# miniufo/xinvert

Measured on AMD Instinct MI355X. Metric: SOR grid-points*iters/sec (fp64) at 3600x1800, masked points counted, higher is better.
Workload: dtype f64

## Files before the change

### xinvert_amd/csrc/xinv_launch.h

```cpp
#pragma once

static inline unsigned cdiv(int64_t a, int64_t b) { return (unsigned)((a + b - 1) / b); }

#if XINV_TEST_HOOKS
static thread_local int *t_hook_record = nullptr;
#endif

struct Plan {
    int path, base, seam, ncol;
    int K, RY, nsg, nrb;
    int nkc, KC;
    bool K2;
    int nsg2, nrb2, nkc2, KC2;
    int joff2;
    int cus;
    int64_t srowf2;
    bool bih_zbe;
    int bih_vm;
    bool aligned;
    unsigned umask;
    unsigned um;
    bool even_split;
    bool nine;
    bool skip;
// ... 355 lines not shown
                if (per) {
                    if (pl.umask) hipLaunchKernelGGL((k_bih_rowclass<true, true>), gb, bb, 0, st, a);
                    else          hipLaunchKernelGGL((k_bih_rowclass<false, true>), gb, bb, 0, st, a);
                } else {
                    if (pl.umask) hipLaunchKernelGGL((k_bih_rowclass<true, false>), gb, bb, 0, st, a);
                    else          hipLaunchKernelGGL((k_bih_rowclass<false, false>), gb, bb, 0, st, a);
                }
            }
            hipLaunchKernelGGL(k_rows_copy_back, dim3(256, (unsigned)nm, 1), dim3(256), 0, st,
                               (const double *)ws->S2, p.sS, p.S, p.sS, p.yc, p.xc,
                               (const XinvCtl *)ws->ctl, m0, 0);
        } else
        for (int cc = 0; cc < pl.ncol; cc++) {
            a.colour = cc;
            if (pl.umask) hipLaunchKernelGGL(k_colour_bih2d<true>, g, b, 0, st, a);
            else          hipLaunchKernelGGL(k_colour_bih2d<false>, g, b, 0, st, a);
        }
    } else if (is3d(p.kind)) {
        ColourArgs3D a;
        memset(&a, 0, sizeof a);
        a.S = p.S; a.sS = p.sS;
        for (int q = 0; q < p.ncoef; q++) { a.c[q] = p.c[q]; a.sc[q] = p.sc[q]; }
        a.zc = p.zc; a.yc = p.yc; a.xc = p.xc;
        a.per = per; a.seam = pl.seam; a.force = 0; a.sc_ = p.sc_; a.ctl = ws->ctl;
        a.nbatch = p.nbatch; a.member0 = m0;
        dim3 b(64, 4, 1);
        dim3 g(cdiv(cdiv(p.xc, 2) + 1, 64), cdiv(p.yc - 2, 4), (unsigned)(nm * (p.zc - 2)));
        for (int pos = 0; pos < pl.ncol; pos++) {
            a.colour = seam_sequence(pos, 2, pl.seam);
            if (p.kind == KIND_GEN3D) hipLaunchKernelGGL(k_colour_gen3d, g, b, 0, st, a);
            else                      hipLaunchKernelGGL(k_colour_std3d, g, b, 0, st, a);
        }
    } else {
        ColourArgs2D a;
        memset(&a, 0, sizeof a);
        a.S = p.S; a.sS = p.sS;
        for (int q = 0; q < p.ncoef; q++) { a.c[q] = p.c[q]; a.sc[q] = p.sc[q]; }
        a.yc = p.yc; a.xc = p.xc;
        a.per = per; a.base = pl.base; a.seam = pl.seam; a.force = 0;
        a.sc_ = p.sc_; a.ctl = ws->ctl; a.member0 = m0;
        dim3 b(64, 4, 1);
        dim3 g(cdiv(cdiv(p.xc, 2) + 1, 64), cdiv(p.yc - 2, 4), (unsigned)nm);
        const bool nine = (pl.base == 4);
        for (int pos = 0; pos < pl.ncol; pos++) {
            a.colour = seam_sequence(pos, pl.base, pl.seam);
            if (p.kind == KIND_STD2D) {
                if (nine) hipLaunchKernelGGL(k_colour_std2d<true>, g, b, 0, st, a);
                else      hipLaunchKernelGGL(k_colour_std2d<false>, g, b, 0, st, a);
            } else if (p.kind == KIND_STD2DT) {
                if (nine) hipLaunchKernelGGL(k_colour_std2dt<true>, g, b, 0, st, a);
                else      hipLaunchKernelGGL(k_colour_std2dt<false>, g, b, 0, st, a);
            } else {
                if (nine) hipLaunchKernelGGL(k_colour_gen2d<true>, g, b, 0, st, a);
                else      hipLaunchKernelGGL(k_colour_gen2d<false>, g, b, 0, st, a);
            }
        }
    }
    NormArgs n;
    n.S = p.S; n.sS = p.sS; n.n = p.zc * p.yc * p.xc; n.undef = p.sc_.undef;
    n.psum = (double *)ws->partials;
    n.pcnt = (long long *)((char *)ws->partials + p.nbatch * XINV_NORM_BLOCKS * sizeof(double));
    n.ctl = ws->ctl; n.stop = p.stop; n.force = 0; n.member0 = m0;
    int nblk = (int)std::min<int64_t>(XINV_NORM_BLOCKS, std::max<int64_t>(1, n.n / 2048));
    hipLaunchKernelGGL(k_norm_partial, dim3(nblk, (unsigned)nm, 1), dim3(256, 1, 1), 0, st, n);
    hipLaunchKernelGGL(k_norm_final, dim3((unsigned)nm, 1, 1), dim3(64, 1, 1), 0, st, n, nblk);
    HIPCHK(hipGetLastError());
    return XINV_OK;
}

static int launch_colour_sweep(const Problem &p, const Plan &pl, Workspace *ws, hipStream_t st)
{
    int64_t chunk = XINV_MEMBER_CHUNK;
    if (is3d(p.kind)) chunk = std::max<int64_t>(1, 65535 / std::max<int64_t>(1, p.zc - 2));
    return for_member_chunks(0, p.nbatch, [&](int64_t m0, int64_t nm) { return launch_colour_chunk(p, pl, ws, st, m0, nm); }, chunk);
}

static int pipe_occ_cap()
{
    return std::max(1, XINV_ENV_INT("XINV_PIPE_OCC", 5));
}

static double tile_cost(int64_t wgs, int64_t rows, int K, int occ, double lone, bool pipe)
{
    return xinv_tile_cost(wgs, rows, K, occ, pipe ? pipe_occ_cap() : 3, lone, pipe ? XINV_PIPE_LAG : 0);
}

static int64_t choose_row_blocks(int64_t yc, int64_t nstrip, int64_t nbatch, int K, int occ, double lone, bool pipe)
{
    return xinv_choose_row_blocks(yc, nstrip, nbatch, K, occ, pipe ? pipe_occ_cap() : 3, lone, pipe ? XINV_PIPE_LAG : 0);
}

static int plan_occ(const Problem &p, const Plan &pl, hipStream_t st, int K, bool *have = nullptr)
{
    const bool ext = (p.BCy == XINV_BC_EXTEND);
    int occ, missing;
    if (p.kind == KIND_BIH2D) {
        FusedBihArgs dummy; memset(&dummy, 0, sizeof dummy);
        occ = 1;
        missing = xinv_launch_fusedbih(false, pl.bih_zbe, pl.bih_vm, dim3(1), st, dummy, &occ);
    } else {
        FusedArgs dummy; memset(&dummy, 0, sizeof dummy);
        occ = pl.nine ? 1 : 2;
        if (pl.nine) missing = xinv_launch_fused9(p.kind == KIND_GEN2D, K, pl.aligned, ext, dim3(1), st, dummy, &occ, pl.seam != 0);
        else if (pl.pipe) missing = xinv_launch_pipe2d(p.kind == KIND_GEN2D, pl.um, pl.npair, pl.pipe_fr, pl.aligned, ext, dim3(1), st, dummy, &occ, 0, pl.seam != 0, pl.fma);
        else missing = fused_dispatch(p.kind, pl.aligned, ext, pl.um | (pl.alias_ac ? 2u : 0u), K, dim3(1), dim3(256), st, dummy, &occ, pl.seam != 0, pl.fma, pl.pq);
    }
    if (have) *have = !missing;
    return occ;
}

static void split_rows_evenly(const Problem &p, Plan &pl, int64_t nrb)
{
    pl.nrb = (int)nrb;
    pl.even_split = true;
    pl.RY = (int)cdiv(p.yc, pl.nrb);
}
static bool rows_per_tile_given(const Problem &p, const xinv_options &opt, Plan &pl)
{
    pl.even_split = false;
    if (opt.rows_per_tile > 0) {
        pl.RY = (opt.rows_per_tile + 1) & ~1;
        pl.nrb = (int)cdiv(p.yc, pl.RY);
    } else if (opt.rows_per_tile < 0)
        split_rows_evenly(p, pl, std::max<int64_t>(1, std::min<int64_t>(-opt.rows_per_tile, p.yc / 2)));
    return opt.rows_per_tile != 0;
}

static int issue_strip_active(const Problem &p, Workspace *ws, hipStream_t st, int UW, int fi)
{
    const int64_t yc = p.yc, nb = p.nbatch;
    const int nstrip = (int)cdiv(p.xc, UW);
    const int64_t cells = yc * nstrip;
    int rc = ensure_dev(&ws->d_act, &ws->d_act_cap, (size_t)(nb * cells));
    if (rc) return rc;
    if ((rc = ensure_pinned(&ws->h_act, &ws->h_act_cap, (size_t)(nb * cells), hipHostMallocDefault))) return rc;
    StripActArgs sa;
    sa.f = p.c[fi]; sa.sf = p.sc[fi]; sa.yc = yc; sa.xc = p.xc; sa.nstrip = nstrip; sa.UW = UW;
    sa.undef = p.sc_.undef; sa.act = ws->d_act;
    hipLaunchKernelGGL(k_strip_active, dim3(cdiv(cells, 4), (unsigned)nb, 1), dim3(256), 0, st, sa);
    HIPCHK(hipMemcpyAsync(ws->h_act, ws->d_act, (size_t)(nb * cells), hipMemcpyDeviceToHost, st));
    ws->act_ready = true; ws->act_uw = UW; ws->act_f = p.c[fi]; ws->act_synced = false;
    return XINV_OK;
}

static int plan_tile_skip(const Problem &p, Plan &pl, Workspace *ws, hipStream_t st,
                          const xinv_options &opt, int fixedRB = 0, int UW_ = 0)
{
    pl.skip = false; pl.ntl = pl.nskip = 0; pl.skip_pct = 0; pl.skip_ppm = 0;
    const bool forced = (opt.flags & XINV_FLAG_FORCE_TILE_SKIP) != 0;
    const int tpw = pl.pipe ? 1 : 4;
    const int K = pl.K, UW = UW_ ? UW_ : strip_uw(pl, K, pl.pipe);
    const int nstrip = (int)cdiv(p.xc, UW);
    const int64_t wscale = 4 / tpw;
    if (!forced && ((int64_t)nstrip * pl.nrb * p.nbatch * wscale < 1024 || (int64_t)nstrip * pl.nrb * wscale < 64 ||
                    p.nbatch > 64))
        return XINV_OK;
    const int64_t yc = p.yc, nb = p.nbatch;
    const int64_t cells = yc * nstrip;
    if (nb * nstrip * (yc + 1) > (int64_t)50000000) return XINV_OK;
    const StreamMap &sm = stream_map(p.kind);
    const int fi = (p.kind == KIND_BIH2D) ? 9 : sm.c[sm.forcing];

    int rc = XINV_OK;
    if (!(ws->act_ready && ws->act_uw == UW && ws->act_f == p.c[fi])) {
        rc = issue_strip_active(p, ws, st, UW, fi);
        if (rc) return rc;
        HIPCHK(hipStreamSynchronize(st));
    } else if (!ws->act_synced)
        HIPCHK(hipStreamSynchronize(st));
    ws->act_ready = false;

    std::vector<int> &pre = ws->h_pre;
    pre.resize((size_t)(nb * nstrip * (yc + 1)));
    int64_t nact = 0;
    for (int64_t m = 0; m < nb; m++) {
        int *q = &pre[(size_t)(m * (yc + 1) * nstrip)];
        for (int s = 0; s < nstrip; s++) q[s] = 0;
        const unsigned char *ha = ws->h_act + m * yc * nstrip;
        for (int64_t r = 0; r < yc; r++, q += nstrip, ha += nstrip)
            for (int s = 0; s < nstrip; s++) q[nstrip + s] = q[s] + ha[s];
        for (int s = 0; s < nstrip; s++) nact += q[s];
    }
    if (!forced && (double)nact > 0.92 * (double)(nb * cells)) return XINV_OK;
    auto rows_active = [&](int64_t m, int strip, int64_t y0, int64_t y1) {
        const int *q = &pre[(size_t)(m * (yc + 1) * nstrip)];
        return q[y1 * nstrip + strip] - q[y0 * nstrip + strip] > 0;
    };

    const bool ext = (p.BCy == XINV_BC_EXTEND);
    auto ntile_ids = [&](int nrb) { return nstrip * nrb; };
    auto id_rb = [&](int, int id) { return id / nstrip; };
    auto tile_active = [&](int64_t m, int nrb, int id) {
        const int rb = id_rb(nrb, id);
        const TileRows t = xinv_tile_rows(id, nstrip, nrb, yc, fixedRB);
        if (t.y0 >= t.y1) return false;
        if (ext && (rb == 0 || rb >= nrb - (fixedRB ? 2 : 1))) return true;
        return rows_active(m, t.strip, t.y0, t.y1);
    };
    auto active_wgs = [&](int nrb, int64_t *maxact) {
        int64_t wgs = 0, mx = 0;
        for (int64_t m = 0; m < nb; m++) {
            int64_t c = 0;
            const int *q = &pre[(size_t)(m * (yc + 1) * nstrip)];
            for (int rb = 0; rb < nrb; rb++) {
                const TileRows t = xinv_tile_rows(rb * nstrip, nstrip, nrb, yc, fixedRB);
                if (t.y0 >= t.y1) continue;
                if (ext && (rb == 0 || rb >= nrb - (fixedRB ? 2 : 1))) { c += nstrip; continue; }
                const int *q0 = q + t.y0 * nstrip, *q1 = q + t.y1 * nstrip;
                for (int st_ = 0; st_ < nstrip; st_++) c += (q1[st_] - q0[st_]) > 0;
            }
            wgs += cdiv(c, tpw); mx = std::max(mx, c);
        }
        if (maxact) *maxact = mx;
        return wgs;
    };
    const int occ = fixedRB ? 2 : plan_occ(p, pl, st, K);
    const bool pp = pl.pipe;
    const double cost0 = tile_cost((int64_t)cdiv((int64_t)nstrip * pl.nrb, tpw) * nb, cdiv(yc, pl.nrb), K, occ, pl.lone, pp);
    int best = pl.nrb; double best_cost = 1e300;
    int lo = pl.nrb, hi = pl.nrb;
    if (!forced && opt.rows_per_tile == 0 && !fixedRB) {
        const int64_t w0 = active_wgs(pl.nrb, nullptr);
        const double share = std::max(0.05, (double)w0 / (double)((int64_t)cdiv((int64_t)nstrip * pl.nrb, tpw) * nb));
        const double centre = (double)pl.nrb / share;
        const int64_t cap_rows = std::max<int64_t>(pl.nrb, yc / 4);
        lo = (int)std::min<int64_t>(cap_rows, std::max<int64_t>(pl.nrb, (int64_t)(centre * 0.85)));
        hi = (int)std::min<int64_t>(cap_rows, std::max<int64_t>(lo, (int64_t)(centre * 1.10) + 1));
    }
    best_cost = tile_cost(active_wgs(pl.nrb, nullptr), cdiv(yc, pl.nrb), K, occ, pl.lone, pp);
    for (int nrb = lo; nrb <= hi; nrb++) {
        const double c = tile_cost(active_wgs(nrb, nullptr), cdiv(yc, nrb), K, occ, pl.lone, pp);
        if (c < best_cost) { best_cost = c; best = nrb; }
    }
    if (!forced && best_cost > 0.95 * cost0) return XINV_OK;

    int64_t maxact = 0;
    active_wgs(best, &maxact);
    const int64_t ntiles = (int64_t)ntile_ids(best);
    const int ntl = (int)(tpw * std::max<int64_t>(1, cdiv(maxact, tpw)));
    int64_t maxskip = 0, nskipped = 0;
    std::vector<std::vector<int>> act((size_t)nb), skp((size_t)nb);
    for (int64_t m = 0; m < nb; m++) {
        for (int id = 0; id < (int)ntiles; id++) {
            const TileRows t = xinv_tile_rows(id, nstrip, best, yc, fixedRB);
            if (t.y0 >= t.y1) continue;
            (tile_active(m, best, id) ? act[(size_t)m] : skp[(size_t)m]).push_back(id);
        }
        maxskip = std::max<int64_t>(maxskip, (int64_t)skp[(size_t)m].size());
        nskipped += (int64_t)skp[(size_t)m].size();
    }
    if (nskipped == 0) return XINV_OK;
    const int nskip = (int)maxskip;
    const size_t nints = (size_t)nb * ((size_t)ntl + nskip);
    rc = ensure_dev(&ws->d_list, &ws->d_list_cap, nints * sizeof(int));
    if (rc) return rc;
    if ((rc = ensure_pinned(&ws->h_list, &ws->h_list_cap, nints * sizeof(int), hipHostMallocDefault))) return rc;
    int *hl = ws->h_list, *hs = ws->h_list + (size_t)nb * ntl;
    for (int64_t m = 0; m < nb; m++) {
        std::vector<int> &am = act[(size_t)m];
        if (pl.seam && !fixedRB) {
            auto heavy = [&](int id) { const int s_ = id % nstrip; return s_ == 0 || s_ == nstrip - 1; };
            const int nh = (int)(std::stable_partition(am.begin(), am.end(), heavy) - am.begin());
            const int nwg = ntl / tpw, q = nwg >> 3, rem = nwg & 7;
            for (int L = 0; L < nwg; L++) {
                const int xcd = L & 7, T = xcd * q + std::min(xcd, rem) + (L >> 3);
                const int sq = xinv_heavy_first(L, nwg, nh / tpw);
                for (int w = 0; w < tpw; w++)
                    hl[m * ntl + T * tpw + w] = sq * tpw + w < (int)am.size() ? am[(size_t)(sq * tpw + w)] : -1;
            }
        } else
        for (int t = 0; t < ntl; t++) hl[m * ntl + t] = t < (int)am.size() ? am[(size_t)t] : -1;
        for (int t = 0; t < nskip; t++) hs[m * nskip + t] = t < (int)skp[(size_t)m].size() ? skp[(size_t)m][t] : -1;
    }
    HIPCHK(hipMemcpyAsync(ws->d_list, ws->h_list, nints * sizeof(int), hipMemcpyHostToDevice, st));
    rc = ensure_dev(&ws->d_tsum, &ws->d_tsum_cap, tsum_layout(nullptr, nb, nskip).bytes);
    if (rc) return rc;
    const TsumPtrs ts = tsum_layout(ws->d_tsum, nb, nskip);
    HIPCHK(hipMemsetAsync(ts.ticket, 0, (size_t)nb * sizeof(unsigned), st));
    SkipNormArgs na;
    na.S = p.S; na.sS = p.sS; na.yc = yc; na.xc = p.xc; na.nstrip = nstrip; na.nrb = best; na.UW = UW; na.RB = fixedRB;
    na.undef = p.sc_.undef; na.skip_list = ws->d_list + (size_t)nb * ntl; na.nskip_max = nskip;
    na.tsum = ts.tsum; na.tcnt = ts.tcnt; na.xsum = ts.xsum; na.xcnt = ts.xcnt; na.ticket = ts.ticket;
    pl.skipna = na;

    pl.skip = true; pl.ntl = ntl; pl.nskip = nskip;
    pl.skip_pct = (int)((100 * nskipped) / (ntiles * nb));
    pl.skip_ppm = (int)((1000000 * nskipped) / (ntiles * nb));
    if (!fixedRB) {
        split_rows_evenly(p, pl, best);
        pl.nsg = (int)cdiv((int64_t)cdiv(p.xc, 128 - (pl.nine ? 8 : 4) * XINV_KMAX - (pl.seam ? 4 : 0)) * pl.nrb, pl.pipe ? 4 : tpw) + 1;
        if (pl.pipe) pl.nsg = std::max(pl.nsg, (int)cdiv(p.xc, UW) * pl.nrb + 1);
    }
    return XINV_OK;
}

static int detect_xuniform(Workspace *ws, hipStream_t st, const double *const *arr,
                           const int64_t *stride, int nstream, int64_t nbatch, int64_t rows,
                           int64_t xc, unsigned *mask)
{
    XUniArgs xa;
    memset(&xa, 0, sizeof xa);
    xa.nstream = nstream;
    for (int q = 0; q < nstream; q++) { xa.c[q] = arr[q]; xa.stride[q] = stride[q]; }
    xa.nbatch = nbatch; xa.yc = rows; xa.xc = xc;
    if (!ws->dflags16) {
        HIPCHK(hipMalloc((void **)&ws->dflags16, 16 * sizeof(int)));
        HIPCHK(hipHostMalloc((void **)&ws->hflags16, 16 * sizeof(int), hipHostMallocDefault));
    }
    xa.flag = ws->dflags16;
    HIPCHK(hipMemsetAsync(ws->dflags16, 0, 16 * sizeof(int), st));
    hipLaunchKernelGGL(k_xuniform, dim3(512, (unsigned)nstream, 1), dim3(256), 0, st, xa);
    HIPCHK(hipMemcpyAsync(ws->hflags16, ws->dflags16, 16 * sizeof(int), hipMemcpyDeviceToHost, st));
    HIPCHK(hipStreamSynchronize(st));
    ws->act_synced = true;
// ... 27 lines not shown
```

### xinvert_amd/csrc/xinv_pipe2d.h

```cpp
#pragma once
#include "xinv_fused.h"

#define XINV_PIPE_P 4
#ifndef XINV_PIPE_B
#define XINV_PIPE_B 2
#endif
#define XINV_PIPE_LAG (XINV_PIPE_B + 5)
#define XINV_PIPE_NS 4
#define XINV_PIPE_UW(np) (128 * (np) - 4 * XINV_PIPE_P)
#ifndef XINV_PIPE_PF0
#define XINV_PIPE_PF0 4
#endif
#ifndef XINV_PIPE_PF
#define XINV_PIPE_PF 4
#endif

template <class M, unsigned UM> struct PipeRec {
    static constexpr int NCO = M::NC - 1;
    static constexpr int NUNI = __builtin_popcount(UM & ((1u << NCO) - 1u));
    static constexpr bool HOIST = M::template hoist<UM>();
    static constexpr int NW = NUNI + (HOIST ? 2 : 0);
    static constexpr int RW = NW == 0 ? 0 : (NW <= 4 ? 4 : 8);
};

// ... 74 lines not shown
        a.q[m * a.n + t] = q;
    }
    if (__any(zero) && (threadIdx.x & 63) == 0) atomicOr(a.flag, 1);
    if (__any(differ) && (threadIdx.x & 63) == 0) atomicOr(a.flag, 2);
}
#endif

__device__ __forceinline__ void xinv_pipe_barrier()
{
    asm volatile("s_waitcnt lgkmcnt(0)\n\ts_barrier" ::: "memory");
}

typedef const double __attribute__((address_space(4))) *xinv_cdouble_ptr;
typedef const char __attribute__((address_space(1))) *xinv_gcptr;
typedef char __attribute__((address_space(1))) *xinv_gptr;
typedef double xinv_v2d __attribute__((ext_vector_type(2)));
typedef const xinv_v2d __attribute__((address_space(1))) *xinv_gcd2ptr;
typedef const double __attribute__((address_space(1))) *xinv_gcdptr;
typedef xinv_v2d __attribute__((address_space(1))) *xinv_gd2ptr;
typedef double __attribute__((address_space(1))) *xinv_gdptr;

__device__ __forceinline__ void pipe_extend_fix(double2 &edge, const double2 &inner, double inner_w,
                                                const LaneCols &lc, bool tall, double u)
{
    if (lc.cls_x == 1) { if (inner.x != u) edge.x = inner.x; }
    else if (lc.cls_x == 2) { if (inner.y != u) edge.x = inner.y; }
    else if (lc.cls_x == 3) {
        if (tall && inner.x != u) edge.x = inner.x;
        if (inner_w != u) edge.x = inner_w;
    }
    if (lc.cls_y == 1) { if (inner.y != u) edge.y = inner.y; }
    else if (lc.cls_y == 3) {
        if (tall && inner.y != u) edge.y = inner.y;
        if (inner.x != u) edge.y = inner.x;
    }
}

template <class M, unsigned UM, bool FR, int NP, bool AL, bool EXT, int PW, int PF, bool SEAM = false>
__device__ __forceinline__ void xinv_pipe_wave(const FusedArgs &a, int64_t m, int yu0, int yu1,
                                               const LaneCols (&lc)[NP], const int64_t (&st0)[NP], int lane,
                                               double2 (*ring)[XINV_PIPE_NS][NP * (FR ? 2 : 1)][XINV_WAVE], int gtot,
                                               double &acc, int &cnt,
                                               unsigned long long seam_lanes = 0ull)
{
    constexpr int P = XINV_PIPE_P, H = 2 * P, D = 4, LAG = XINV_PIPE_LAG, B = XINV_PIPE_B;
    constexpr int R = PF + D;
    constexpr int PFR = M::PIPE_PFR;
    using REC = PipeRec<M, UM>;
    constexpr int NC = M::NC, FQ = M::NC - 1, RW = REC::RW;
    constexpr bool HOIST = REC::HOIST;
    constexpr int RS = FR ? 2 : 1;
    static_assert(R % D == 0 && R % B == 0 && R % XINV_PIPE_NS == 0,
                  "the unroll period must keep row parity, ring slots and barriers compile-time");
    const int ycr = (int)a.yc;
    const unsigned rowbytes = (unsigned)a.xc * 8u;
    const double u = a.sc_.undef;
    const int slice_bytes = (int)(rowbytes * (unsigned)ycr);
    const __amdgpu_buffer_rsrc_t rsS = __builtin_amdgcn_make_buffer_rsrc((void *)(a.src + m * a.sS), 0, slice_bytes, 0x00020000);
    const __amdgpu_buffer_rsrc_t rsD = __builtin_amdgcn_make_buffer_rsrc((void *)(a.dst + m * a.sS), 0, slice_bytes, 0x00020000);
    __amdgpu_buffer_rsrc_t rsC[NC];
#pragma unroll
    for (int q = 0; q < NC; q++)
        rsC[q] = __builtin_amdgcn_make_buffer_rsrc((void *)(a.c[q] + m * a.sc[q]), 0, slice_bytes, 0x00020000);
    const xinv_cdouble_ptr rowf = (xinv_cdouble_ptr)(uintptr_t)(reinterpret_cast<const double *>(a.rowf) + m * a.yc * RW);
    unsigned lo0[NP], lo1[NP], so0[NP], so1[NP];
#pragma unroll
    for (int q = 0; q < NP; q++) {
        lo0[q] = (unsigned)lc[q].l0 * 8u; lo1[q] = (unsigned)lc[q].l1 * 8u;
        so0[q] = lc[q].use_x ? (unsigned)st0[q] * 8u : 0xffffffffu;
        so1[q] = lc[q].use_y ? (unsigned)(st0[q] + 1) * 8u : 0xffffffffu;
    }

    unsigned long long okx64[NP], oky64[NP];
    double nsx[NP], nsy[NP];
    int nnx[NP], nny[NP];
#pragma unroll
    for (int q = 0; q < NP; q++) {
        okx64[q] = __builtin_amdgcn_ballot_w64(lc[q].ok_x) & ~seam_lanes; oky64[q] = __builtin_amdgcn_ballot_w64(lc[q].ok_y);
        nsx[q] = nsy[q] = 0.0; nnx[q] = nny[q] = 0;
    }
    static_assert(!SEAM || (NP == 1 && !AL && PipeRec<M, UM>::HOIST),
                  "seam variants: one column pair per lane, per-row records, updates under EXEC masks");

    const int in_lo = yu0 - H + 2 * PW;
    const int in_hi = yu1 - 1 + H - 2 * PW;

    double2 sw[NP][R];
    CoefWin<NC, R> cw[NP];
    double rokw[R];
#pragma unroll
    for (int t = 0; t < R; t++) {
        rokw[t] = 0.0;
#pragma unroll
        for (int q = 0; q < NP; q++) {
            sw[q][t] = make_double2(0.0, 0.0);
            cw[q].rq[t] = 0.0; cw[q].mx[t] = 0u; cw[q].my[t] = 0u;
#pragma unroll
            for (int c = 0; c < NC; c++) { cw[q].v[c][t] = make_double2(0.0, 0.0); cw[q].s[c][t] = 0.0; }
        }
    }

    const int maxo = (int)(rowbytes * (unsigned)(ycr - 1));
    int nxo = (yu0 - H + 2 * PW) * (int)rowbytes;
    int nxr = (yu0 - H + 2 * PW) * (RW * 8);
    auto ldrow = [&](__amdgpu_buffer_rsrc_t rs, int soff, auto qtag) {
        constexpr int q = decltype(qtag)::value;
        double2 v;
        if (AL) {
            const auto t = __builtin_amdgcn_raw_buffer_load_b128(rs, (int)lo0[q], soff, 0);
            v.x = __hiloint2double((int)t[1], (int)t[0]); v.y = __hiloint2double((int)t[3], (int)t[2]);
        } else {
            const auto t0 = __builtin_amdgcn_raw_buffer_load_b64(rs, (int)lo0[q], soff, 0);
            const auto t1 = __builtin_amdgcn_raw_buffer_load_b64(rs, (int)lo1[q], soff, 0);
            v.x = __hiloint2double((int)t0[1], (int)t0[0]); v.y = __hiloint2double((int)t1[1], (int)t1[0]);
        }
        return v;
    };
    auto request = [&](int, auto stag) {
        constexpr int slot = decltype(stag)::value;
        const int soff = min(max(nxo, 0), maxo);
        nxo += (int)rowbytes;
        asm("" : "+s"(nxo));
        xinv_unroll_steps([&](auto qtag) {
            constexpr int q = decltype(qtag)::value;
            if (PW == 0) sw[q][slot] = ldrow(rsS, soff, qtag);
            xinv_unroll_steps([&](auto ctag) {
                constexpr int c = decltype(ctag)::value;
                if (!((UM >> c) & 1u) && !(FR && c == FQ && PW > 0)) cw[q].v[c][slot] = ldrow(rsC[c], soff, qtag);
            }, std::make_integer_sequence<int, NC>{});
        }, std::make_integer_sequence<int, NP>{});
    };
    auto request_rf = [&](int, auto stag) {
        constexpr int slot = decltype(stag)::value;
        if constexpr (RW > 0) {
            const unsigned roff = (unsigned)min(max(nxr, 0), (ycr - 1) * (RW * 8));
            nxr += RW * 8;
            const xinv_cdouble_ptr pr = (xinv_cdouble_ptr)((const char __attribute__((address_space(4))) *)rowf + roff);
            double rec[RW];
#pragma unroll
            for (int k = 0; k < RW; k++) rec[k] = pr[k];
#pragma unroll
            for (int q = 0; q < NP; q++) {
                int k = 0;
#pragma unroll
                for (int c = 0; c < NC - 1; c++)
                    if ((UM >> c) & 1u) cw[q].s[c][slot] = rec[k++];
                if (HOIST) { cw[q].rq[slot] = rec[k]; rokw[slot] = rec[k + 1]; }
            }
        }
    };
    xinv_unroll_steps([&](auto ttag) { request(in_lo + decltype(ttag)::value, ttag); asm volatile("" ::: "memory"); },
                      std::make_integer_sequence<int, PF>{});
    xinv_unroll_steps([&](auto ttag) { request_rf(in_lo + decltype(ttag)::value, ttag); },
                      std::make_integer_sequence<int, PFR>{});

    auto half_pass = [&](auto xtag, auto jtag, auto ptag, auto mtag, auto fixt) {
        constexpr int X = decltype(xtag)::value, sj = decltype(jtag)::value, sjp = decltype(ptag)::value,
                      sjm = decltype(mtag)::value;
        constexpr bool FIX = decltype(fixt)::value;
        static_assert(!FIX || (X == 0 && NP == 1), "column xc-1 sits in an .x slot");
        const double edge = (X == 0) ? xinv_lane_up(sw[NP - 1][sj].y) : xinv_lane_down(sw[0][sj].x);
        double nv[NP];
#pragma unroll
        for (int q = 0; q < NP; q++) {
            double w, e;
            if (X == 0) { w = (q == 0) ? edge : sw[q > 0 ? q - 1 : 0][sj].y; e = sw[q][sj].y; }
            else        { w = sw[q][sj].x; e = (q == NP - 1) ? edge : sw[q < NP - 1 ? q + 1 : q][sj].x; }
            if constexpr (FIX) e = xinv_lane_down(sw[q][sj].x);
            const double t = M::template inc<X, UM, R, false>(cw[q], sj, sjp, comp<X>(sw[q][sj]), comp<X>(sw[q][sjp]),
                                              comp<X>(sw[q][sjm]), w, e, a.sc_);
            if constexpr (HOIST) {
                const unsigned long long rm = (FIX ? seam_lanes : (X ? oky64[q] : okx64[q])) &
                                              (unsigned long long)__double_as_longlong(rokw[sj]);
                if constexpr (ModelFma<M>::value)
                    nv[q] = xinv_fma_where_ne(comp<X>(sw[q][sj]), t, cw[q].rq[sj], comp<X>(cw[q].v[FQ][sj]), u, rm);
                else
                    nv[q] = xinv_add_where_ne(comp<X>(sw[q][sj]), t, comp<X>(cw[q].v[FQ][sj]), u, rm);
            } else {
                const unsigned long long pm = __builtin_amdgcn_ballot_w64((X ? cw[q].my[sj] : cw[q].mx[sj]) != 0u);
                nv[q] = xinv_add_where(comp<X>(sw[q][sj]), t, pm);
            }
        }
#pragma unroll
        for (int q = 0; q < NP; q++) setc<X>(sw[q][sj], nv[q]);
    };
    auto half_sweep = [&](auto xtag, auto jtag, auto ptag, auto mtag) {
        constexpr int X = decltype(xtag)::value;
        half_pass(xtag, jtag, ptag, mtag, std::false_type{});
        if constexpr (SEAM && X == 0) {
            constexpr int sj = decltype(jtag)::value;
            half_pass(xtag, jtag, ptag, mtag, std::true_type{});
            sw[0][sj].y = xinv_bitsel64(seam_lanes, sw[0][sj].x, sw[0][sj].y);
        }
    };

    int g = 0;
#pragma unroll
    for (; g < LAG * PW; g++) {
        if (PW > 0 && g == LAG * PW - 1) {
#pragma unroll
            for (int q = 0; q < NP; q++) {
                sw[q][0] = ring[PW - 1][(2 * PW) % XINV_PIPE_NS][q * RS][lane];
                if (FR) cw[q].v[FQ][0] = ring[PW - 1][(2 * PW) % XINV_PIPE_NS][q * RS + 1][lane];
            }
        }
        if ((g + 1) % B == 0) xinv_pipe_barrier();
    }

    for (int rb_ = in_lo; rb_ <= in_hi; rb_ += R) {
        xinv_unroll_steps([&](auto utag) {
            constexpr int U = decltype(utag)::value;
            constexpr int X = (U & 1) ? 0 : 1;
#define SLOT(w) ((U - (w) + 4 * R) % R)
#define RSLOT(w) ((2 * PW + U - (w) + 64 * XINV_PIPE_NS) % XINV_PIPE_NS)
#define ITAG(v) std::integral_constant<int, (v)>{}
            const int r = rb_ + U;
            request(r + PF, ITAG((U + PF) % R));
            request_rf(r + PFR, ITAG((U + PFR) % R));
            if (PW > 0) {
#pragma unroll
                for (int q = 0; q < NP; q++) {
                    sw[q][(U + 1) % R] = ring[PW - 1][RSLOT(-1)][q * RS][lane];
                    if (FR) cw[q].v[FQ][(U + 1) % R] = ring[PW - 1][RSLOT(-1)][q * RS + 1][lane];
                }
            }
            if constexpr (!HOIST) {
                const bool rv = (r - 1 >= 1) && (r - 1 <= ycr - 2);
#pragma unroll
                for (int q = 0; q < NP; q++)
                    M::template derive<UM, R, false>(cw[q], SLOT(0), SLOT(1), rv && lc[q].ok_x, rv && lc[q].ok_y, a.sc_);
            }
            {
                const int ja = r - 1;
                constexpr int sj = SLOT(1), sjp = SLOT(0), sjm = SLOT(2);
                if (EXT) {
                    if (ja == 1 || ja == ycr - 2) {
                        const double wl = xinv_lane_up(sw[NP - 1][sj].y);
#pragma unroll
                        for (int q = 0; q < NP; q++) {
                            const double iw = (q == 0) ? wl : sw[q > 0 ? q - 1 : 0][sj].y;
                            if (ja == 1) pipe_extend_fix(sw[q][sjm], sw[q][sj], iw, lc[q], a.tall, u);
                            if (ja == ycr - 2) pipe_extend_fix(sw[q][sjp], sw[q][sj], iw, lc[q], a.tall, u);
                        }
                    }
                }
                half_sweep(ITAG(X), ITAG(sj), ITAG(sjp), ITAG(sjm));
            }
            {
                const int jb = r - 2;
                constexpr int sj = SLOT(2), sjp = SLOT(1), sjm = SLOT(3);
                half_sweep(ITAG(X), ITAG(sj), ITAG(sjp), ITAG(sjm));
                if ((unsigned)(jb - yu0) < (unsigned)(yu1 - yu0)) {
#pragma unroll
                    for (int q = 0; q < NP; q++) {
                        const double2 t = sw[q][sj];
                        xinv_norm_row(nsx[q], nsy[q], nnx[q], nny[q], t.x, t.y, u);
                    }
                }
                if (PW < P - 1) {
#pragma unroll
                    for (int q = 0; q < NP; q++) {
                        ring[PW][RSLOT(2)][q * RS][lane] = sw[q][sj];
                        if (FR) ring[PW][RSLOT(2)][q * RS + 1][lane] = cw[q].v[FQ][sj];
                    }
                } else if ((unsigned)(jb - yu0) < (unsigned)(yu1 - yu0)) {
                    const int doff = jb * (int)rowbytes;
                    xinv_unroll_steps([&](auto qtag) {
                        constexpr int q = decltype(qtag)::value;
                        const double2 t = sw[q][sj];
                        typedef unsigned xinv_v4u __attribute__((__vector_size__(16)));
                        typedef unsigned xinv_v2u __attribute__((__vector_size__(8)));
                        if (AL) {
                            const xinv_v4u tv = {(unsigned)__double2loint(t.x), (unsigned)__double2hiint(t.x),
                                                 (unsigned)__double2loint(t.y), (unsigned)__double2hiint(t.y)};
                            __builtin_amdgcn_raw_buffer_store_b128(tv, rsD, (int)so0[q], doff, 0);
                        } else {
                            const xinv_v2u tx = {(unsigned)__double2loint(t.x), (unsigned)__double2hiint(t.x)};
                            const xinv_v2u ty = {(unsigned)__double2loint(t.y), (unsigned)__double2hiint(t.y)};
                            __builtin_amdgcn_raw_buffer_store_b64(tx, rsD, (int)so0[q], doff, 0);
                            __builtin_amdgcn_raw_buffer_store_b64(ty, rsD, (int)so1[q], doff, 0);
                        }
                    }, std::make_integer_sequence<int, NP>{});
                }
            }
            if ((LAG * PW + U + 1) % B == 0) xinv_pipe_barrier();
#undef SLOT
#undef RSLOT
#undef ITAG
        }, std::make_integer_sequence<int, R>{});
        g += R;
    }
    for (; g < gtot; g++) if ((g + 1) % B == 0) xinv_pipe_barrier();
#pragma unroll
    for (int q = 0; q < NP; q++) {
        acc += (lc[q].use_x ? nsx[q] : 0.0);
        acc += (lc[q].use_y ? nsy[q] : 0.0);
        cnt += (lc[q].use_x ? nnx[q] : 0) + (lc[q].use_y ? nny[q] : 0);
    }
}

template <class M, unsigned UM, bool FR, int NP, bool AL, bool EXT, bool SEAM = false>
__global__ __launch_bounds__(64 * XINV_PIPE_P) void k_pipe2d(FusedArgs a_)
{
    xinv_fresh_scalar_cache();
    constexpr int P = XINV_PIPE_P, K = P, H = 2 * K, LAG = XINV_PIPE_LAG, B = XINV_PIPE_B;
    __shared__ double2 ring[P - 1][XINV_PIPE_NS][NP * (FR ? 2 : 1)][XINV_WAVE];

    unsigned tag;
    int T;
    double acc = 0.0;
    int cnt = 0;
    const int wave = threadIdx.x >> 6, lane = threadIdx.x & 63;
    int pwi;
    {
    const FusedArgs &a = a_;
    const int64_t m = a.member0 + blockIdx.y;
    XinvCtl *ctl = a.ctl + m;
    if (!a.force && xinv_ctl_done(ctl)) return;
    if (a.lag && (int)blockIdx.x == a.nwg) { xinv_lag_reduce_prev(a, ctl, m); return; }
    tag = a.lag ? a.tag : xinv_ctl_seq(ctl);

    const int NB = a.nwg;
    {
        const int L = blockIdx.x, q = NB >> 3, rem = NB & 7, xcd = L & 7, idx = L >> 3;
        T = xcd * q + (xcd < rem ? xcd : rem) + idx;
    }
    pwi = (wave + (int)(blockIdx.x >> 8)) & (P - 1);
    int wt = T;
    bool active = wt < a.nstrip * a.nrb;
    if constexpr (SEAM) {
        if (!a.tile_list && NB == a.nstrip * a.nrb)
            wt = xinv_seam_tile(xinv_heavy_first((int)blockIdx.x, NB, (a.nstrip == 1 ? 1 : 2) * a.nrb), a.nstrip, a.nrb);
    }
    if (a.tile_list) {
        wt = a.tile_list[m * a.ntl + T];
        active = wt >= 0;
        wt = active ? wt : 0;
    }
    int rb = wt / a.nstrip, strip = wt - rb * a.nstrip;
    const int64_t xc = a.xc, yc = a.yc;
    int yu0, yu1;
    if (a.RY > 0) {
        yu0 = rb * a.RY;
        yu1 = (yu0 + a.RY < (int)yc) ? yu0 + a.RY : (int)yc;
    } else {
        yu0 = (int)((((int64_t)rb * yc) / a.nrb) & ~(int64_t)1);
        yu1 = (rb + 1 == a.nrb) ? (int)yc : (int)((((int64_t)(rb + 1) * yc) / a.nrb) & ~(int64_t)1);
    }
    const int UW = SEAM ? xinv_ring_uw(xc, H) : XINV_PIPE_UW(NP), HW = SEAM ? xinv_ring_hw(xc, H, strip) : H;
    const int64_t xu0 = (int64_t)strip * UW;
    LaneCols lc[NP];
    int64_t st0[NP];
    RingSeam rs = {0ull, false};
#pragma unroll
    for (int q = 0; q < NP; q++) {
        if constexpr (SEAM) lc[q] = make_lanecols_ring(xu0, HW, UW, lane, xc, rs);
        else lc[q] = make_lanecols<AL>(xu0, H, UW, lane, xc, a.per != 0, NP, q);
        st0[q] = xu0 - HW + 2 * NP * lane + 2 * q;
    }

    if (active) {
        const int ry = yu1 - yu0;
        int gtot = 0;
#pragma unroll
        for (int pw = 0; pw < P; pw++) {
            const int per = (pw == 0 ? XINV_PIPE_PF0 : XINV_PIPE_PF) + 4;
            const int n = ry + 2 * H - 4 * pw;
            const int g = LAG * pw + ((n + per - 1) / per) * per;
            gtot = g > gtot ? g : gtot;
        }
        gtot = ((gtot + B - 1) / B) * B;
        const bool wraps = rs.any;
#define XINV_PIPE_MARCH(SM) \
        switch (pwi) { \
        case 0: xinv_pipe_wave<M, UM, FR, NP, AL, EXT, 0, XINV_PIPE_PF0, SM>(a, m, yu0, yu1, lc, st0, lane, ring, gtot, acc, cnt, rs.lanes); break; \
        case 1: xinv_pipe_wave<M, UM, FR, NP, AL, EXT, 1, XINV_PIPE_PF, SM>(a, m, yu0, yu1, lc, st0, lane, ring, gtot, acc, cnt, rs.lanes); break; \
        case 2: xinv_pipe_wave<M, UM, FR, NP, AL, EXT, 2, XINV_PIPE_PF, SM>(a, m, yu0, yu1, lc, st0, lane, ring, gtot, acc, cnt, rs.lanes); break; \
        default: xinv_pipe_wave<M, UM, FR, NP, AL, EXT, 3, XINV_PIPE_PF, SM>(a, m, yu0, yu1, lc, st0, lane, ring, gtot, acc, cnt, rs.lanes); break; \
        }
        if (wraps) { XINV_PIPE_MARCH(SEAM) } else { XINV_PIPE_MARCH(false) }
#undef XINV_PIPE_MARCH
    }
    }
    const FusedArgs __attribute__((address_space(4))) *kp =
        (const FusedArgs __attribute__((address_space(4))) *)__builtin_amdgcn_kernarg_segment_ptr();
    asm volatile("" : "+s"(kp) :: "memory");
    if (kp->no_ctl) return;
    const int64_t m = kp->member0 + blockIdx.y;
    XinvCtl *ctl = kp->ctl + m;
    const int NB = kp->nwg;
    struct { unsigned long long *psum; const double *xsum; const long long *xcnt; int lag; XinvStop stop; const void *hook; } a;
    a.psum = kp->psum; a.xsum = kp->xsum; a.xcnt = kp->xcnt; a.lag = kp->lag;
    a.hook = XINV_TEST_HOOKS ? (const void *)kp->dbg : nullptr;
    a.stop.mxLoop = kp->stop.mxLoop; a.stop.tolerance = kp->stop.tolerance;
    a.stop.stop_on_zero_norm = kp->stop.stop_on_zero_norm;

    {
        unsigned long long *pw = a.psum + (size_t)m * XINV_KMAX * NB * XINV_PW;
        const double ws = xinv_wave_sum(acc);
        const long long wc = xinv_wave_sum_ll((long long)cnt);
        if (lane == 0 && !xinv_hook_withhold(a.hook, T, tag, m)) {
            const unsigned long long hi = (unsigned long long)tag << 32;
            const unsigned long long bits = (unsigned long long)__double_as_longlong(ws);
            unsigned long long *q = pw + ((size_t)pwi * NB + T) * XINV_PW;
            __hip_atomic_store(q + 0, hi | (bits & 0xffffffffull), __ATOMIC_RELAXED, __HIP_MEMORY_SCOPE_AGENT);
            __hip_atomic_store(q + 1, hi | (bits >> 32), __ATOMIC_RELAXED, __HIP_MEMORY_SCOPE_AGENT);
            __hip_atomic_store(q + 2, hi | (unsigned long long)(unsigned)wc, __ATOMIC_RELAXED,
                               __HIP_MEMORY_SCOPE_AGENT);
        }
        if (a.lag || blockIdx.x != gridDim.x - 1) return;
        __syncthreads();
        xinv_norm_reduce<K, P>(wave, lane, NB, tag, pw, ctl, a.stop, a.xsum ? a.xsum[m] : 0.0,
                               a.xcnt ? a.xcnt[m] : 0);
    }
}
```

### xinvert_amd/csrc/xinv_tiles.h

```cpp
#pragma once
#include <cstdint>
#ifndef __HIPCC__
#ifndef __host__
#define __host__
#endif
#ifndef __device__
#define __device__
#endif
#endif

struct TileRows { int strip; int64_t y0, y1; };
__host__ __device__ inline TileRows xinv_tile_rows(int wt, int nstrip, int nrb, int64_t yc, int RY)
{
    TileRows t;
    const int rb = wt / nstrip;
    t.strip = wt - rb * nstrip;
    if (RY > 0) { t.y0 = (int64_t)rb * RY; t.y1 = (t.y0 + RY < yc) ? t.y0 + RY : yc; }
    else {
        t.y0 = (((int64_t)rb * yc) / nrb) & ~(int64_t)1;
        t.y1 = (rb + 1 == nrb) ? yc : ((((int64_t)(rb + 1) * yc) / nrb) & ~(int64_t)1);
    }
    return t;
}

// ... 14 lines not shown
    const int k = s - nh, nl = nstrip > edges ? nstrip - edges : 1, rb = k / nl;
    return rb * nstrip + (k - rb * nl) + 1;
}

__host__ __device__ inline bool xinv_ring_asym(int64_t xc, int H) { return xc >= (int64_t)(128 - 2 * H - 2) + H; }
__host__ __device__ inline int xinv_ring_uw(int64_t xc, int H) { return 128 - 2 * H - (xinv_ring_asym(xc, H) ? 2 : 4); }
__host__ __device__ inline int xinv_ring_hw(int64_t xc, int H, int strip)
{
    return xinv_ring_asym(xc, H) ? (strip == 0 ? H + 2 : H) : H + 2;
}

__host__ __device__ inline int xinv_p3_slot_tile(int L, int nfull, int nkc, int &kc)
{
    int g;
    kc = 0;
    if (L < nfull) g = L;
    else { const int q = L - nfull; g = nfull + q / nkc; kc = q - (g - nfull) * nkc; }
    return g;
}
__host__ __device__ inline bool xinv_p3_slot_reduces(int L, int nfull, int nkc, int NT, int ml)
{
    const int gl = (ml + 1) * NT - 1;
    return (gl < nfull) ? (L == gl) : (L == nfull + (gl - nfull) * nkc + nkc - 1);
}
__host__ __device__ inline int xinv_p3_slot_member_tile(int L, int nfull, int NT, int ml, int g)
{
    if (L < nfull) {
        const int L0 = ml * NT;
        const int n = (L0 + NT <= nfull) ? NT : (nfull - L0);
        const int xcd = L & 7;
        auto below = [](int e, int x) { return (e >> 3) * x + ((e & 7) < x ? (e & 7) : x); };
        auto same = [](int e, int x) { return e <= x ? 0 : ((e - x + 7) >> 3); };
        return (below(L0 + n, xcd) - below(L0, xcd)) + (same(L, xcd) - same(L0, xcd));
    }
    return g - ml * NT;
}
struct P3Slot { int ml, Tj, kc; bool whole, reducer; };
__host__ __device__ inline P3Slot xinv_p3_slot(int L, int nfull, int nkc, int NT)
{
    P3Slot s;
    s.whole = L < nfull;
    const int g = xinv_p3_slot_tile(L, nfull, nkc, s.kc);
    s.ml = g / NT;
    s.reducer = xinv_p3_slot_reduces(L, nfull, nkc, NT, s.ml);
    s.Tj = xinv_p3_slot_member_tile(L, nfull, NT, s.ml, g);
    return s;
}

__host__ inline int64_t xinv_p3_whole_tiles(int64_t tiles, int nk, int64_t KC, int64_t zc, int cus_, double *cost_out = nullptr)
{
    const bool no_rem = cus_ < 0;
    const int64_t cus = cus_ < 0 ? -cus_ : cus_;
    auto cdiv64 = [](int64_t a, int64_t b) { return (a + b - 1) / b; };
    const double cf = (double)(zc + 4), cs = (double)(KC + 14);
    double best = (double)cdiv64(tiles, cus) * cf;
    int64_t nfull = tiles;
    if (nk > 1) {
        const double call = (double)cdiv64(tiles * nk, cus) * cs;
        if (call < best * 0.97) { best = call; nfull = 0; }
        const int64_t r = tiles % cus, R = tiles / cus;
        if (r && R && !no_rem) {
            const double crem = (double)R * cf + (double)cdiv64(r * nk, cus) * cs;
            if (crem < best * 0.985) { best = crem; nfull = tiles - r; }
        }
    }
    if (cost_out) *cost_out = best;
    return nfull;
}

__host__ __device__ inline bool xinv_p3_extend_ok(int64_t yc, int joff, int RJ, int H, int RR)
{
    if ((H + joff) % RR == RR - 1) return false;
    const int64_t jbo = (yc - 1 + joff) / RJ;
    auto together = [&](int64_t jb) { return ((yc - 2) - (jb * RJ - H - joff)) % RR != RR - 1; };
    if (!together(jbo)) return false;
    if (jbo > 0 && (yc - 1 + joff) - jbo * RJ <= 1 && !together(jbo - 1)) return false;
    return true;
}
__host__ __device__ inline int xinv_p3_extend_joff(int64_t yc, int RJ, int H, int RR)
{
    return xinv_p3_extend_ok(yc, 0, RJ, H, RR) ? 0 : (xinv_p3_extend_ok(yc, 2, RJ, H, RR) ? 2 : -1);
}

__host__ inline int64_t xinv_cdiv(int64_t a, int64_t b) { return (a + b - 1) / b; }

__host__ inline double xinv_tile_cost(int64_t wgs, int64_t rows, int K, int occ, int occ_cap, double lone, int pipe_lag)
{
    const bool pipe = pipe_lag > 0;
    occ = occ < occ_cap ? occ : occ_cap;
    occ = occ > 1 ? occ : 1;
    const int64_t cap = 256 * (int64_t)occ, period = pipe ? 4 : 2 * K + 2;
    const int64_t steps = pipe ? xinv_cdiv(rows + 1 + 4 + 3 * pipe_lag, 8) * 8
                               : xinv_cdiv(rows + 1 + 4 * K, period) * period;
    const int64_t r = xinv_cdiv(wgs, cap), rounds = r > 1 ? r : 1;
    const int64_t w_last = wgs - (rounds - 1) * cap;
    const double full = pipe ? 1.5 + occ : ((occ == 1) ? lone : (double)occ);
    const double last = pipe ? 1.5 + (double)xinv_cdiv(w_last, 256) : ((w_last <= 256) ? lone : (double)xinv_cdiv(w_last, 256));
    return ((double)(rounds - 1) * full + last) * (double)steps;
}

__host__ inline int64_t xinv_choose_row_blocks(int64_t yc, int64_t nstrip, int64_t nbatch, int K, int occ, int occ_cap,
                                               double lone, int pipe_lag)
{
    const bool pipe = pipe_lag > 0;
    int64_t best = 1; double best_cost = 1e300;
    const int64_t n0 = xinv_cdiv(yc, pipe ? 512 : 128), nmin = n0 > 1 ? n0 : 1, nmax = nmin > yc / 4 ? nmin : yc / 4;
    for (int64_t nr = nmin; nr <= nmax; nr++) {
        const int64_t wgs = xinv_cdiv(nstrip * nr, pipe ? 1 : 4) * nbatch;
        const double cost = xinv_tile_cost(wgs, xinv_cdiv(yc, nr), K, occ, occ_cap, lone, pipe_lag);
        if (cost <= best_cost * 1.0001) { best_cost = cost < best_cost ? cost : best_cost; best = nr; }
    }
    return best;
}

__host__ inline int64_t xinv_k_chunk_planes(int64_t zc, int nk) { return xinv_cdiv(xinv_cdiv(zc, nk), 4) * 4; }
template <class Cost>
__host__ inline int xinv_choose_k_chunks(int64_t zc, Cost cost)
{
    int best = 1; double best_cost = 1e300;
    for (int nk = 1; nk <= 16; nk++) {
        const int64_t KC = xinv_k_chunk_planes(zc, nk);
        if (nk > 1 && (KC < 16 || (int64_t)(nk - 1) * KC >= zc)) break;
        const double c = cost(nk, KC);
        if (c < best_cost * 0.97) { best_cost = c; best = nk; }
    }
    return best;
}
__host__ inline int xinv_k_chunks_fused3d(int64_t zc, int64_t wgs)
{
    return xinv_choose_k_chunks(zc, [&](int nk, int64_t KC) { return (double)xinv_cdiv(wgs * nk, 256) * (double)(KC + (nk > 1 ? 10 : 2)); });
}
__host__ inline int xinv_k_chunks_pipe3d(int64_t zc, int64_t tiles, int cus)
{
    return xinv_choose_k_chunks(zc, [&](int nk, int64_t KC) { double c; xinv_p3_whole_tiles(tiles, nk, KC, zc, cus, &c); return c; });
}
```

Before: 752.2 billion.

## Trim pipeline prologue padding per wave and model exact pipe steps in tile cost

The pipelined 2D SOR kernel now shifts each wave's start row so that the padding needed to round its row count up to the unroll period is taken out of the start-up lag instead of being added as idle steps. Ring-buffer slots are flipped to match the shifted start. The total step count is computed by a shared helper. The host tile-cost model now uses this exact step count and the tallest even-split tile height, so row-block selection matches the kernel's real schedule. This is meant to cut wasted prologue and epilogue steps, at the cost of more complex index arithmetic with some risk of off-by-one errors in the ring-slot mapping.

```diff
diff --git a/xinvert_amd/csrc/xinv_launch.h b/xinvert_amd/csrc/xinv_launch.h
--- a/xinvert_amd/csrc/xinv_launch.h
+++ b/xinvert_amd/csrc/xinv_launch.h
@@ -461,12 +461,14 @@
 
 static double tile_cost(int64_t wgs, int64_t rows, int K, int occ, double lone, bool pipe)
 {
-    return xinv_tile_cost(wgs, rows, K, occ, pipe ? pipe_occ_cap() : 3, lone, pipe ? XINV_PIPE_LAG : 0);
+    return xinv_tile_cost(wgs, rows, K, occ, pipe ? pipe_occ_cap() : 3, lone, pipe ? XINV_PIPE_LAG : 0, pipe ? XINV_PIPE_B : 0,
+                          XINV_PIPE_PF0 + 4, XINV_PIPE_PF + 4);
 }
 
 static int64_t choose_row_blocks(int64_t yc, int64_t nstrip, int64_t nbatch, int K, int occ, double lone, bool pipe)
 {
-    return xinv_choose_row_blocks(yc, nstrip, nbatch, K, occ, pipe ? pipe_occ_cap() : 3, lone, pipe ? XINV_PIPE_LAG : 0);
+    return xinv_choose_row_blocks(yc, nstrip, nbatch, K, occ, pipe ? pipe_occ_cap() : 3, lone, pipe ? XINV_PIPE_LAG : 0,
+                                  pipe ? XINV_PIPE_B : 0, XINV_PIPE_PF0 + 4, XINV_PIPE_PF + 4);
 }
 
 static int plan_occ(const Problem &p, const Plan &pl, hipStream_t st, int K, bool *have = nullptr)
@@ -595,7 +597,11 @@
     };
     const int occ = fixedRB ? 2 : plan_occ(p, pl, st, K);
     const bool pp = pl.pipe;
-    const double cost0 = tile_cost((int64_t)cdiv((int64_t)nstrip * pl.nrb, tpw) * nb, cdiv(yc, pl.nrb), K, occ, pl.lone, pp);
+    auto cost_rows = [&](int nrb) -> int64_t {
+        if (!pp) return cdiv(yc, nrb);
+        return pl.even_split ? xinv_even_split_tallest(yc, nrb) : std::min<int64_t>(pl.RY, yc);
+    };
+    const double cost0 = tile_cost((int64_t)cdiv((int64_t)nstrip * pl.nrb, tpw) * nb, cost_rows(pl.nrb), K, occ, pl.lone, pp);
     int best = pl.nrb; double best_cost = 1e300;
     int lo = pl.nrb, hi = pl.nrb;
     if (!forced && opt.rows_per_tile == 0 && !fixedRB) {
@@ -606,9 +612,9 @@
         lo = (int)std::min<int64_t>(cap_rows, std::max<int64_t>(pl.nrb, (int64_t)(centre * 0.85)));
         hi = (int)std::min<int64_t>(cap_rows, std::max<int64_t>(lo, (int64_t)(centre * 1.10) + 1));
     }
-    best_cost = tile_cost(active_wgs(pl.nrb, nullptr), cdiv(yc, pl.nrb), K, occ, pl.lone, pp);
+    best_cost = tile_cost(active_wgs(pl.nrb, nullptr), cost_rows(pl.nrb), K, occ, pl.lone, pp);
     for (int nrb = lo; nrb <= hi; nrb++) {
-        const double c = tile_cost(active_wgs(nrb, nullptr), cdiv(yc, nrb), K, occ, pl.lone, pp);
+        const double c = tile_cost(active_wgs(nrb, nullptr), cost_rows(nrb), K, occ, pl.lone, pp);
         if (c < best_cost) { best_cost = c; best = nrb; }
     }
     if (!forced && best_cost > 0.95 * cost0) return XINV_OK;
diff --git a/xinvert_amd/csrc/xinv_pipe2d.h b/xinvert_amd/csrc/xinv_pipe2d.h
--- a/xinvert_amd/csrc/xinv_pipe2d.h
+++ b/xinvert_amd/csrc/xinv_pipe2d.h
@@ -180,8 +180,15 @@
     static_assert(!SEAM || (NP == 1 && !AL && PipeRec<M, UM>::HOIST),
                   "seam variants: one column pair per lane, per-row records, updates under EXEC masks");
 
-    const int in_lo = yu0 - H + 2 * PW;
+    const int front = xinv_pipe_front(yu1 - yu0, PW, LAG, R);
+    const int in_lo = yu0 + xinv_pipe_first_row(yu1 - yu0, PW, LAG, R);
     const int in_hi = yu1 - 1 + H - 2 * PW;
+    typedef double2 (*ring_t)[XINV_PIPE_NS][NP * (FR ? 2 : 1)][XINV_WAVE];
+    static_assert(XINV_PIPE_NS == 4 && (XINV_PIPE_P - 1) * sizeof(ring[0]) <= 65536, "ring offsets as ds immediates");
+    const int flip = PW > 0 ? xinv_pipe_slot_flip(front) : 0;
+    const ring_t ring_lo = (ring_t)(&ring[0][flip]);
+    const ring_t ring_hi = (ring_t)(&ring[0][2 - flip]);
+#define RING(pw_, name_) ((name_) < 2 ? ring_lo : ring_hi)[pw_][(name_) & 1]
 
     double2 sw[NP][R];
     CoefWin<NC, R> cw[NP];
@@ -199,8 +206,8 @@
     }
 
     const int maxo = (int)(rowbytes * (unsigned)(ycr - 1));
-    int nxo = (yu0 - H + 2 * PW) * (int)rowbytes;
-    int nxr = (yu0 - H + 2 * PW) * (RW * 8);
+    int nxo = in_lo * (int)rowbytes;
+    int nxr = in_lo * (RW * 8);
     auto ldrow = [&](__amdgpu_buffer_rsrc_t rs, int soff, auto qtag) {
         constexpr int q = decltype(qtag)::value;
         double2 v;
@@ -292,17 +299,17 @@
         }
     };
 
+    const int gread = xinv_pipe_first_read(yu1 - yu0, PW, LAG, R);
     int g = 0;
-#pragma unroll
-    for (; g < LAG * PW; g++) {
-        if (PW > 0 && g == LAG * PW - 1) {
-#pragma unroll
-            for (int q = 0; q < NP; q++) {
-                sw[q][0] = ring[PW - 1][(2 * PW) % XINV_PIPE_NS][q * RS][lane];
-                if (FR) cw[q].v[FQ][0] = ring[PW - 1][(2 * PW) % XINV_PIPE_NS][q * RS + 1][lane];
-            }
+    for (; g < gread; g++) if ((g + 1) % B == 0) xinv_pipe_barrier();
+    if (PW > 0 && gread >= 0) {
+#pragma unroll
+        for (int q = 0; q < NP; q++) {
+            sw[q][0] = RING(PW - 1, (2 * PW) % XINV_PIPE_NS)[q * RS][lane];
+            if (FR) cw[q].v[FQ][0] = RING(PW - 1, (2 * PW) % XINV_PIPE_NS)[q * RS + 1][lane];
         }
         if ((g + 1) % B == 0) xinv_pipe_barrier();
+        g++;
     }
 
     for (int rb_ = in_lo; rb_ <= in_hi; rb_ += R) {
@@ -318,8 +325,8 @@
             if (PW > 0) {
 #pragma unroll
                 for (int q = 0; q < NP; q++) {
-                    sw[q][(U + 1) % R] = ring[PW - 1][RSLOT(-1)][q * RS][lane];
-                    if (FR) cw[q].v[FQ][(U + 1) % R] = ring[PW - 1][RSLOT(-1)][q * RS + 1][lane];
+                    sw[q][(U + 1) % R] = RING(PW - 1, RSLOT(-1))[q * RS][lane];
+                    if (FR) cw[q].v[FQ][(U + 1) % R] = RING(PW - 1, RSLOT(-1))[q * RS + 1][lane];
                 }
             }
             if constexpr (!HOIST) {
@@ -358,8 +365,8 @@
                 if (PW < P - 1) {
 #pragma unroll
                     for (int q = 0; q < NP; q++) {
-                        ring[PW][RSLOT(2)][q * RS][lane] = sw[q][sj];
-                        if (FR) ring[PW][RSLOT(2)][q * RS + 1][lane] = cw[q].v[FQ][sj];
+                        RING(PW, RSLOT(2))[q * RS][lane] = sw[q][sj];
+                        if (FR) RING(PW, RSLOT(2))[q * RS + 1][lane] = cw[q].v[FQ][sj];
                     }
                 } else if ((unsigned)(jb - yu0) < (unsigned)(yu1 - yu0)) {
                     const int doff = jb * (int)rowbytes;
@@ -389,6 +396,7 @@
         g += R;
     }
     for (; g < gtot; g++) if ((g + 1) % B == 0) xinv_pipe_barrier();
+#undef RING
 #pragma unroll
     for (int q = 0; q < NP; q++) {
         acc += (lc[q].use_x ? nsx[q] : 0.0);
@@ -458,16 +466,7 @@
     }
 
     if (active) {
-        const int ry = yu1 - yu0;
-        int gtot = 0;
-#pragma unroll
-        for (int pw = 0; pw < P; pw++) {
-            const int per = (pw == 0 ? XINV_PIPE_PF0 : XINV_PIPE_PF) + 4;
-            const int n = ry + 2 * H - 4 * pw;
-            const int g = LAG * pw + ((n + per - 1) / per) * per;
-            gtot = g > gtot ? g : gtot;
-        }
-        gtot = ((gtot + B - 1) / B) * B;
+        const int gtot = xinv_pipe_gtot(yu1 - yu0, LAG, B, XINV_PIPE_PF0 + 4, XINV_PIPE_PF + 4);
         const bool wraps = rs.any;
 #define XINV_PIPE_MARCH(SM) \
         switch (pwi) { \
diff --git a/xinvert_amd/csrc/xinv_tiles.h b/xinvert_amd/csrc/xinv_tiles.h
--- a/xinvert_amd/csrc/xinv_tiles.h
+++ b/xinvert_amd/csrc/xinv_tiles.h
@@ -120,16 +120,68 @@
     return xinv_p3_extend_ok(yc, 0, RJ, H, RR) ? 0 : (xinv_p3_extend_ok(yc, 2, RJ, H, RR) ? 2 : -1);
 }
 
+__host__ __device__ inline int xinv_pipe_rows(int ry, int pw) { return ry + 16 - 4 * pw; }
+__host__ __device__ inline int xinv_pipe_pad(int ry, int pw, int period)
+{
+    return (period - xinv_pipe_rows(ry, pw) % period) % period;
+}
+__host__ __device__ inline int xinv_pipe_front(int ry, int pw, int lag, int period)
+{
+    const int pad = xinv_pipe_pad(ry, pw, period), room = lag * pw;
+    return (pad < room ? pad : room) & ~1;
+}
+__host__ __device__ inline int xinv_pipe_end(int ry, int pw, int lag, int period)
+{
+    return xinv_pipe_pad(ry, pw, period) - xinv_pipe_front(ry, pw, lag, period);
+}
+__host__ __device__ inline int xinv_pipe_first_row(int ry, int pw, int lag, int period)
+{
+    return -8 + 2 * pw - xinv_pipe_front(ry, pw, lag, period);
+}
+__host__ __device__ inline int xinv_pipe_start(int ry, int pw, int lag, int period)
+{
+    return lag * pw - xinv_pipe_front(ry, pw, lag, period);
+}
+__host__ __device__ inline int xinv_pipe_first_read(int ry, int pw, int lag, int period)
+{
+    return xinv_pipe_start(ry, pw, lag, period) - 1;
+}
+__host__ __device__ inline int xinv_pipe_slot_flip(int front) { return front & 2; }
+__host__ __device__ inline int xinv_pipe_gtot(int ry, int lag, int b, int period0, int period)
+{
+    int gtot = 0;
+    for (int pw = 0; pw < 4; pw++) {
+        const int per = pw == 0 ? period0 : period;
+        const int g = xinv_pipe_start(ry, pw, lag, per) + xinv_pipe_rows(ry, pw) + xinv_pipe_pad(ry, pw, per);
+        gtot = g > gtot ? g : gtot;
+    }
+    return ((gtot + b - 1) / b) * b;
+}
+
 __host__ inline int64_t xinv_cdiv(int64_t a, int64_t b) { return (a + b - 1) / b; }
 
-__host__ inline double xinv_tile_cost(int64_t wgs, int64_t rows, int K, int occ, int occ_cap, double lone, int pipe_lag)
+__host__ inline int64_t xinv_even_split_tallest(int64_t yc, int64_t nrb)
+{
+    const int64_t D = 2 * nrb, q = yc / D, s = yc - q * D;
+    const int64_t last = 2 * (q + s / 2 - ((nrb - 1) * s) / D) + (s & 1);
+    const int64_t inner = nrb > 1 ? 2 * (q + ((nrb - 1) * s >= D ? 1 : 0)) : 0;
+    return last > inner ? last : inner;
+}
+
+__host__ inline int64_t xinv_tile_steps(int64_t rows, int K, int pipe_lag, int pipe_b = 0, int pipe_per0 = 8, int pipe_per = 8)
+{
+    if (pipe_lag > 0 && pipe_b > 0) return xinv_pipe_gtot((int)rows, pipe_lag, pipe_b, pipe_per0, pipe_per);
+    const int64_t period = 2 * K + 2;
+    return pipe_lag > 0 ? xinv_cdiv(rows + 1 + 4 + 3 * pipe_lag, 8) * 8 : xinv_cdiv(rows + 1 + 4 * K, period) * period;
+}
+__host__ inline double xinv_tile_cost(int64_t wgs, int64_t rows, int K, int occ, int occ_cap, double lone, int pipe_lag,
+                                      int pipe_b = 0, int pipe_per0 = 8, int pipe_per = 8)
 {
     const bool pipe = pipe_lag > 0;
     occ = occ < occ_cap ? occ : occ_cap;
     occ = occ > 1 ? occ : 1;
-    const int64_t cap = 256 * (int64_t)occ, period = pipe ? 4 : 2 * K + 2;
-    const int64_t steps = pipe ? xinv_cdiv(rows + 1 + 4 + 3 * pipe_lag, 8) * 8
-                               : xinv_cdiv(rows + 1 + 4 * K, period) * period;
+    const int64_t cap = 256 * (int64_t)occ;
+    const int64_t steps = xinv_tile_steps(rows, K, pipe_lag, pipe_b, pipe_per0, pipe_per);
     const int64_t r = xinv_cdiv(wgs, cap), rounds = r > 1 ? r : 1;
     const int64_t w_last = wgs - (rounds - 1) * cap;
     const double full = pipe ? 1.5 + occ : ((occ == 1) ? lone : (double)occ);
@@ -138,14 +190,15 @@
 }
 
 __host__ inline int64_t xinv_choose_row_blocks(int64_t yc, int64_t nstrip, int64_t nbatch, int K, int occ, int occ_cap,
-                                               double lone, int pipe_lag)
+                                               double lone, int pipe_lag, int pipe_b = 0, int pipe_per0 = 8, int pipe_per = 8)
 {
     const bool pipe = pipe_lag > 0;
     int64_t best = 1; double best_cost = 1e300;
     const int64_t n0 = xinv_cdiv(yc, pipe ? 512 : 128), nmin = n0 > 1 ? n0 : 1, nmax = nmin > yc / 4 ? nmin : yc / 4;
     for (int64_t nr = nmin; nr <= nmax; nr++) {
         const int64_t wgs = xinv_cdiv(nstrip * nr, pipe ? 1 : 4) * nbatch;
-        const double cost = xinv_tile_cost(wgs, xinv_cdiv(yc, nr), K, occ, occ_cap, lone, pipe_lag);
+        const int64_t rows = (pipe && pipe_b > 0) ? xinv_even_split_tallest(yc, nr) : xinv_cdiv(yc, nr);
+        const double cost = xinv_tile_cost(wgs, rows, K, occ, occ_cap, lone, pipe_lag, pipe_b, pipe_per0, pipe_per);
         if (cost <= best_cost * 1.0001) { best_cost = cost < best_cost ? cost : best_cost; best = nr; }
     }
     return best;
```

Result: faster. 773.2 billion (median of 6 runs) (+2.8%).
